# google/vizier

Measured on AMD Instinct MI355X. Metric: suggest_wall_clock_ms_gp_bandit_20d_n1000, lower is better.
Workload: dtype fp32; 1 GPU; model=gp_bandit_matern52_ucb_eagle, dim=20, n_trials=1000, acquisition_evals_per_gpu=75000, eagle_batch=25, ard=warm_lbfgs_12it_x2, global_batch=1, parallelism=dp1_sharded_sweep

## Files before the change

### vizier_amd/_src/ops/csrc/eagle_sweep.hip

```cpp

#include <hip/hip_runtime.h>

#include "common.h"

#define BLOCK 256
#define MAX_POOL 128
#define SWEEP_NCHUNK 10
#define POOL_LDS_CAP 8192
#define RESIDENT_CAP (POOL_LDS_CAP / 2)

__device__ __forceinline__ float cload(const float* p) {
  return __hip_atomic_load(p, __ATOMIC_RELAXED, __HIP_MEMORY_SCOPE_AGENT);
}
__device__ __forceinline__ void cstore(float* p, float v) {
  __hip_atomic_store(p, v, __ATOMIC_RELAXED, __HIP_MEMORY_SCOPE_AGENT);
}

__device__ __forceinline__ void grid_sync(unsigned int* bar,
                                          unsigned int& target) {
  __builtin_amdgcn_s_waitcnt(0);
  __syncthreads();
  target += gridDim.x;
  if (threadIdx.x == 0) {
    asm volatile("" ::: "memory");
    const unsigned int count = __hip_atomic_fetch_add(
        bar, 1u, __ATOMIC_RELAXED, __HIP_MEMORY_SCOPE_AGENT) + 1u;
    if ((int)(count - target) < 0) {
      while ((int)(__hip_atomic_load(bar, __ATOMIC_RELAXED,
                                     __HIP_MEMORY_SCOPE_AGENT) -
                   target) < 0) {
        __builtin_amdgcn_s_sleep(8);
      }
    }
    asm volatile("" ::: "memory");
  }
  __syncthreads();
}

#define FOLD_MAX_TILES 1024

__device__ __forceinline__ void reduce_all_partials(
    const float* var_ws, int batch_size, int total_tiles, float* wp) {
  const int tid = threadIdx.x;
  float sacc[VZ_QF_QMAX];
#pragma unroll
  for (int q = 0; q < VZ_QF_QMAX; ++q) sacc[q] = 0.0f;
  for (int w0 = 0; w0 < total_tiles; w0 += BLOCK) {
    const int w = w0 + tid;
    const bool live = w < total_tiles;
    const int wc = live ? w : total_tiles - 1;
    float v[VZ_QF_QMAX];
#pragma unroll
    for (int q = 0; q < VZ_QF_QMAX; ++q) {
      const int qc = min(q, batch_size - 1);
      v[q] = cload(var_ws + (long)qc * (total_tiles + 1) + wc);
    }
#pragma unroll
    for (int q = 0; q < VZ_QF_QMAX; ++q) {
      sacc[q] = live ? sacc[q] + v[q] : sacc[q];
    }
  }
  const int lane = tid & (WAVE_SIZE - 1);
#pragma unroll
  for (int off = WAVE_SIZE / 2; off > 1; off >>= 1) {
    const bool up = (lane & off) != 0;
#pragma unroll
    for (int i = 0; i < off / 2; ++i) {
      const float keep = up ? sacc[2 * i + 1] : sacc[2 * i];
      const float send = up ? sacc[2 * i] : sacc[2 * i + 1];
      sacc[i] = keep + __shfl_xor(send, off, WAVE_SIZE);
    }
  }
  const float total = sacc[0] + __shfl_xor(sacc[0], 1, WAVE_SIZE);
  if ((lane & 1) == 0) {
    const int q = (int)(__brev((unsigned)(lane >> 1)) >> 27);
    wp[(tid / WAVE_SIZE) * VZ_QF_QMAX + q] = total;
  }
}

__device__ __forceinline__ float fold_quad(const float* wp, int q) {
  return (wp[q] + wp[2 * VZ_QF_QMAX + q]) +
         (wp[VZ_QF_QMAX + q] + wp[3 * VZ_QF_QMAX + q]);
}

template <typename LoadK, typename StoreP>
__device__ __forceinline__ void vz_quadform_tile_pipelined(
    const float* __restrict__ kinv, int b, int n, int tile, int tiles_n,
    float* k_i_lds, float* k_j_lds, LoadK loadk, StoreP store,
    unsigned long long* prof = nullptr) {
  constexpr int kStage = VZ_QF_QMAX * VZ_QF_TILE / BLOCK;
  const int tid = threadIdx.x;
  const bool profme = (prof != nullptr && tid == 0);
  unsigned long long tq0 = profme ? wall_clock64() : 0;
  const int ti = tile / tiles_n, tj = tile % tiles_n;
  const int i0 = ti * VZ_QF_TILE, j0 = tj * VZ_QF_TILE;
  const int ilen = min(VZ_QF_TILE, n - i0);
  const int jlen = min(VZ_QF_TILE, n - j0);
  {
    const int c = tid % VZ_QF_TILE;
    const int q0 = tid / VZ_QF_TILE;
    const int ci = i0 + min(c, ilen - 1), cj = j0 + min(c, jlen - 1);
    float ri[kStage], rj[kStage];
#pragma unroll
    for (int u = 0; u < kStage; ++u) {
      const long base =
          (long)min(q0 + u * (BLOCK / VZ_QF_TILE), b - 1) * n;
      ri[u] = loadk(base + ci);
      rj[u] = loadk(base + cj);
    }
#pragma unroll
    for (int u = 0; u < kStage; ++u) {
      const bool inq = q0 + u * (BLOCK / VZ_QF_TILE) < b;
      k_i_lds[tid + u * BLOCK] = (inq && c < ilen) ? ri[u] : 0.0f;
      k_j_lds[tid + u * BLOCK] = (inq && c < jlen) ? rj[u] : 0.0f;
    }
  }
  __syncthreads();
  if (profme) {
    const unsigned long long tq1 = wall_clock64();
    prof[0] += tq1 - tq0;
    tq0 = tq1;
  }
  const int wave = tid / WAVE_SIZE;
  const int lane = tid % WAVE_SIZE;
  float acc[8];
#pragma unroll
  for (int qq = 0; qq < 8; ++qq) acc[qq] = 0.0f;
  if (lane < jlen) {
    if (ilen == VZ_QF_TILE) {
      for (int ib = 0; ib < VZ_QF_TILE; ib += 8) {
        float kvv[8];
#pragma unroll
        for (int u = 0; u < 8; ++u) {
          kvv[u] = kinv[(long)(i0 + ib + u) * n + j0 + lane];
        }
#pragma unroll
        for (int u = 0; u < 8; ++u) {
#pragma unroll
          for (int qq = 0; qq < 8; ++qq) {
            acc[qq] = fmaf(
                k_i_lds[(wave * 8 + qq) * VZ_QF_TILE + ib + u],
                kvv[u], acc[qq]);
          }
        }
      }
    } else {
      for (int i = 0; i < ilen; ++i) {
        const float kv = kinv[(long)(i0 + i) * n + j0 + lane];
#pragma unroll
        for (int qq = 0; qq < 8; ++qq) {
          acc[qq] = fmaf(k_i_lds[(wave * 8 + qq) * VZ_QF_TILE + i], kv,
                         acc[qq]);
        }
      }
    }
  }
#pragma unroll
  for (int qq = 0; qq < 8; ++qq) {
    const int q = wave * 8 + qq;
    float v = acc[qq] * k_j_lds[q * VZ_QF_TILE + lane];
    v = wave_reduce_sum(v);
    if (lane == 0 && q < b) store(q, v);
  }
  __syncthreads();
  if (profme) prof[1] += wall_clock64() - tq0;
}

__device__ __forceinline__ float sweep_matern52(float d2) {
#pragma clang fp contract(off)
  const float r = sqrtf(fmaxf(d2, 0.0f));
  const float sr = 2.2360679774997896f * r;
  const float one_sr = 1.0f + sr;
  return fmaf(sr * sr, 1.0f / 3.0f, one_sr) * __expf(-sr);
}

#define KV_ROWS 4
#define KV_CHUNK 4

template <bool VEC4>
__device__ __forceinline__ void sweep_kvec(
    const float* __restrict__ x, const float* __restrict__ inv_ls,
    const float* __restrict__ alpha, const float* xq_lds, float* k_row,
    int dc, int n, float amp2, float& mu_acc, float& min_linf) {
  for (int row0 = threadIdx.x; row0 < n; row0 += KV_ROWS * BLOCK) {
    const float* xr[KV_ROWS];
    float al[KV_ROWS];
#pragma unroll
    for (int s = 0; s < KV_ROWS; ++s) {
      const int rc = min(row0 + s * BLOCK, n - 1);
      xr[s] = x + (long)rc * dc;
      al[s] = alpha[rc];
    }
    auto load_chunk = [&](float (&buf)[KV_ROWS][KV_CHUNK], int j0) {
#pragma unroll
      for (int s = 0; s < KV_ROWS; ++s) {
        if (VEC4) {
          const float4 v = *reinterpret_cast<const float4*>(xr[s] + j0);
          buf[s][0] = v.x; buf[s][1] = v.y; buf[s][2] = v.z; buf[s][3] = v.w;
        } else {
#pragma unroll
          for (int c = 0; c < KV_CHUNK; ++c) {
            buf[s][c] = xr[s][min(j0 + c, dc - 1)];
          }
        }
      }
    };
    float d2[KV_ROWS], linf[KV_ROWS];
#pragma unroll
    for (int s = 0; s < KV_ROWS; ++s) d2[s] = linf[s] = 0.0f;
    for (int j0 = 0; j0 < dc; j0 += KV_CHUNK) {
      float cur[KV_ROWS][KV_CHUNK];
      load_chunk(cur, j0);
      float xq[KV_CHUNK], il[KV_CHUNK];
#pragma unroll
      for (int c = 0; c < KV_CHUNK; ++c) {
        const int jc = VEC4 ? j0 + c : min(j0 + c, dc - 1);
        xq[c] = xq_lds[jc];
        il[c] = inv_ls[jc];
      }
#pragma unroll
      for (int c = 0; c < KV_CHUNK; ++c) {
        if (VEC4 || j0 + c < dc) {
#pragma unroll
          for (int s = 0; s < KV_ROWS; ++s) {
            const float diff = xq[c] - cur[s][c];
            const float z = diff * il[c];
            d2[s] = fmaf(z, z, d2[s]);
            linf[s] = fmaxf(linf[s], fabsf(diff));
          }
        }
      }
    }
#pragma unroll
    for (int s = 0; s < KV_ROWS; ++s) {
      const int row = row0 + s * BLOCK;
      const bool live = row < n;
      const float kv = amp2 * sweep_matern52(d2[s]);
      if (live) cstore(k_row + row, kv);
      mu_acc = live ? fmaf(kv, al[s], mu_acc) : mu_acc;
      min_linf = live ? fminf(min_linf, linf[s]) : min_linf;
    }
  }
}

extern "C" __global__ __launch_bounds__(BLOCK) void
eagle_sweep_kernel(
    float* __restrict__ pool_cont,
    float* __restrict__ rewards,
    float* __restrict__ perturbations,
    float* __restrict__ best_reward,
    unsigned long long* __restrict__ iter_ptr,
    unsigned int* __restrict__ barrier_buf,
    const float* __restrict__ x,
    const float* __restrict__ inv_ls,
    const float* __restrict__ alpha,
    const float* __restrict__ kinv,
    float* __restrict__ out_cont,
    float* __restrict__ k_ws,
    float* __restrict__ mu_ws,
    float* __restrict__ dist_ws,
    float* __restrict__ var_ws,
    float* __restrict__ slot_ws,
    int n_batches, int batch_size, int pool_size, int dc, int n,
    long long it_start, long long iterations,
    float visibility, float gravity, float neg_gravity, float norm_scale,
    float penalize_factor, float perturbation_lower_bound,
    float base_perturbation,
    unsigned long long seed_suggest, unsigned long long seed_update,
    float amp2, float mean_c, int acq, float coef, float best_value,
    float tr_radius) {
  __shared__ float scale[MAX_POOL];
  __shared__ float red[8];
  __shared__ float s_scalar;
  __shared__ __attribute__((aligned(16))) float xq_lds[512];
  __shared__ float pool_lds[POOL_LDS_CAP];
  __shared__ float st_rewards[MAX_POOL];
  __shared__ float st_perts[MAX_POOL];
  __shared__ float st_best;

  const int tid = threadIdx.x;
  const int G = gridDim.x;
  const int pool_elems = pool_size * dc;
  const bool resident = pool_elems <= RESIDENT_CAP;
  const bool stage_pool = !resident && pool_elems <= POOL_LDS_CAP;
  const bool pool_in_lds = resident || stage_pool;
  const bool owner = blockIdx.x < batch_size;
  const bool x_vec4 = dc % KV_CHUNK == 0 &&
                      (reinterpret_cast<unsigned long long>(x) & 15) == 0;
  float* st_pool = pool_lds + RESIDENT_CAP;
  const float* pl = resident ? st_pool : pool_lds;
  auto fsum = [](float a, float c) { return a + c; };
  auto fmin_ = [](float a, float c) { return fminf(a, c); };
  auto fmax_ = [](float a, float c) { return fmaxf(a, c); };

  const bool profwg = (blockIdx.x == 0 && threadIdx.x == 0);
  unsigned long long tmark = profwg ? wall_clock64() : 0;
  unsigned int bar_target = 0;
#define VZ_SWEEP_PROF(slot)                                        \
  if (profwg) {                                                    \
    const unsigned long long tnow = wall_clock64();                \
    iter_ptr[2 + (slot)] += tnow - tmark;                          \
    tmark = tnow;                                                  \
  }

  if (resident && owner) {
    for (int e = tid; e < pool_elems; e += BLOCK) st_pool[e] = pool_cont[e];
    for (int p = tid; p < pool_size; p += BLOCK) {
      st_rewards[p] = rewards[p];
      st_perts[p] = perturbations[p];
    }
    if (tid == 0) st_best = best_reward[0];
    __syncthreads();
  }

  for (long long it = it_start; it < it_start + iterations; ++it) {
    const unsigned long long offset = (unsigned long long)it;
    float* slot_c = slot_ws + (long)(it & 1) * batch_size * (dc + 2);
    float* slot_mu = slot_c + batch_size * dc;
    float* slot_dist = slot_mu + batch_size;
    const int batch_start =
        (int)(offset % (unsigned long long)n_batches) * batch_size;
    if (profwg) tmark = wall_clock64();

    for (int b = blockIdx.x; b < batch_size; b += G) {
      if (stage_pool) {
        for (int e = tid; e < pool_elems; e += BLOCK) {
          pool_lds[e] = cload(pool_cont + e);
        }
        __syncthreads();
      }
      const int me = batch_start + b;
      const float my_reward = resident ? st_rewards[me]
                                       : cload(rewards + me);
      const float my_pert = resident ? st_perts[me]
                                     : cload(perturbations + me);
      for (int p = tid; p < pool_size; p += BLOCK) {
        float d2 = 0.0f;
        if (pool_in_lds) {
          for (int j = 0; j < dc; ++j) {
            const float diff = pl[me * dc + j] - pl[p * dc + j];
            d2 = fmaf(diff, diff, d2);
          }
        } else {
          for (int j = 0; j < dc; ++j) {
            const float diff = cload(pool_cont + me * dc + j) -
                               cload(pool_cont + p * dc + j);
            d2 = fmaf(diff, diff, d2);
          }
        }
        const float reward_p = resident ? st_rewards[p]
                                        : cload(rewards + p);
        const float dir = (reward_p - my_reward >= 0.0f) ? gravity
                                                         : -neg_gravity;
        const float force = __expf(-visibility * d2 / dc * 10.0f);
        float s = dir * force;
        if (!isfinite(reward_p)) s = 0.0f;
        scale[p] = s;
      }
      __syncthreads();
      float pulls = 0.0f, pushes = 0.0f;
      for (int p = tid; p < pool_size; p += BLOCK) {
        pulls += (scale[p] > 0.0f) ? 1.0f : 0.0f;
        pushes += (scale[p] < 0.0f) ? 1.0f : 0.0f;
      }
      float n_pull = block_reduce(pulls, red, fsum, 0.0f);
      if (tid == 0) red[4] = fmaxf(n_pull, 1.0f);
      __syncthreads();
      float n_push = block_reduce(pushes, red, fsum, 0.0f);
      if (tid == 0) red[5] = fmaxf(n_push, 1.0f);
      __syncthreads();
      const float inv_pull = 1.0f / red[4];
      const float inv_push = 1.0f / red[5];
      float ssum = 0.0f;
      for (int p = tid; p < pool_size; p += BLOCK) {
        const float s = scale[p];
        const float ns = norm_scale * (s > 0.0f ? s * inv_pull
                                                : s * inv_push);
        scale[p] = ns;
        ssum += ns;
      }
      __syncthreads();
      float scale_sum = block_reduce(ssum, red, fsum, 0.0f);
      if (tid == 0) s_scalar = scale_sum;
      __syncthreads();
      scale_sum = s_scalar;
      for (int j = tid; j < dc; j += BLOCK) {
        float moved = 0.0f;
        if (pool_in_lds) {
          for (int p = 0; p < pool_size; ++p) {
            moved = fmaf(scale[p], pl[p * dc + j], moved);
          }
        } else {
          for (int p = 0; p < pool_size; ++p) {
            moved = fmaf(scale[p], cload(pool_cont + p * dc + j), moved);
          }
        }
        const float mine = pool_in_lds ? pl[me * dc + j]
                                       : cload(pool_cont + me * dc + j);
        moved = mine + (moved - mine * scale_sum);
        float noise = vz_rng_laplace<float>(seed_suggest, offset,
                                     (unsigned)(b * dc + j));
        noise = (noise >= 0.0f) ? 1.0f : -1.0f;
        const float cand = moved + noise * my_pert;
        out_cont[b * dc + j] = cand;
        if (resident) cstore(slot_c + b * dc + j, cand);
        xq_lds[j] = cand;
      }
      __syncthreads();

      float mu_acc = 0.0f;
      float min_linf = INFINITY;
      if (x_vec4) {
        sweep_kvec<true>(x, inv_ls, alpha, xq_lds, k_ws + (long)b * n, dc,
                         n, amp2, mu_acc, min_linf);
      } else {
        sweep_kvec<false>(x, inv_ls, alpha, xq_lds, k_ws + (long)b * n, dc,
                          n, amp2, mu_acc, min_linf);
      }
      float mu = block_reduce(mu_acc, red, fsum, 0.0f);
      if (tid == 0) {
        cstore(mu_ws + b, mu);
        if (resident) cstore(slot_mu + b, mu);
      }
      __syncthreads();
      float dist = block_reduce(min_linf, red, fmin_, INFINITY);
      if (tid == 0) {
        cstore(dist_ws + b, dist);
        if (resident) cstore(slot_dist + b, dist);
      }
      __syncthreads();
    }
    VZ_SWEEP_PROF(0)
    grid_sync(barrier_buf, bar_target);
    VZ_SWEEP_PROF(1)

    {
      const int tiles_n = (n + VZ_QF_TILE - 1) / VZ_QF_TILE;
      const int total_tiles = tiles_n * tiles_n;
      float* k_i_lds = pool_lds;
      float* k_j_lds = pool_lds + VZ_QF_QMAX * VZ_QF_TILE;
      for (int tile = blockIdx.x; tile < total_tiles; tile += G) {
        const int t = tile;
        vz_quadform_tile_pipelined(
            kinv, batch_size, n, t, tiles_n, k_i_lds, k_j_lds,
            [&](long idx) { return cload(k_ws + idx); },
            [&](int q, float v) {
              cstore(var_ws + (long)q * (total_tiles + 1) + t, v);
            },
            blockIdx.x == 0 ? iter_ptr + 10 : nullptr);
      }
    }
    VZ_SWEEP_PROF(2)
    grid_sync(barrier_buf, bar_target);
    VZ_SWEEP_PROF(3)

    const int tiles_n_c = (n + VZ_QF_TILE - 1) / VZ_QF_TILE;
    const int total_tiles_c = tiles_n_c * tiles_n_c;
    const bool fold = total_tiles_c <= FOLD_MAX_TILES;
    if (!fold) {
      for (int q = blockIdx.x; q < batch_size; q += G) {
        float sacc = 0.0f;
        for (int w = tid; w < total_tiles_c; w += BLOCK) {
          sacc += cload(var_ws + (long)q * (total_tiles_c + 1) + w);
        }
        float total = block_reduce(sacc, red, fsum, 0.0f);
        if (tid == 0) {
          cstore(var_ws + (long)q * (total_tiles_c + 1) + total_tiles_c,
                 total);
        }
        __syncthreads();
      }
      VZ_SWEEP_PROF(4)
      grid_sync(barrier_buf, bar_target);
      VZ_SWEEP_PROF(5)
    }

    float* wp = pool_lds;
    float* sc_lds = pool_lds + 4 * VZ_QF_QMAX;
    auto score_of = [&](float quad, float mu_raw, float dist) {
      float var = fmaxf(amp2 - quad, 1e-12f);
      const float sd = sqrtf(var);
      const float mu = mu_raw + mean_c;
      return vz_trust_region(vz_acq_score(acq, mu, sd, coef, best_value),
                             dist, tr_radius);
    };
    if (resident) {
      if (owner) {
        float mu_t = 0.0f, dist_t = 0.0f;
        if (tid < batch_size) {
          mu_t = cload(slot_mu + tid);
          dist_t = cload(slot_dist + tid);
        }
        if (fold) {
          reduce_all_partials(var_ws, batch_size, total_tiles_c, wp);
        }
        __syncthreads();
        if (tid < WAVE_SIZE) {
          float score = -INFINITY;
          if (tid < batch_size) {
            float* reduced =
                var_ws + (long)tid * (total_tiles_c + 1) + total_tiles_c;
            float quad;
            if (fold) {
              quad = fold_quad(wp, tid);
              if (tid % G == (int)blockIdx.x) cstore(reduced, quad);
            } else {
              quad = cload(reduced);
            }
            score = score_of(quad, mu_t, dist_t);
            sc_lds[tid] = score;
          }
          const float batch_max = wave_reduce_max(score);
          if (tid == 0) s_scalar = fmaxf(st_best, batch_max);
        }
        __syncthreads();
        const float new_best = s_scalar;
        for (int e = tid; e < batch_size * dc; e += BLOCK) {
          const int i = e / dc;
          const int me = batch_start + i;
          const int ej = me * dc + (e - i * dc);
          const float new_r = sc_lds[i];
          const float old_r = st_rewards[me];
          const bool improved = new_r > old_r;
          const float old_pert = st_perts[me];
          const float pert = improved ? old_pert
                                      : old_pert * penalize_factor;
          const float reward = improved ? new_r : old_r;
          const bool dead = (pert < perturbation_lower_bound) &&
                            (reward != new_best);
          if (dead) {
            st_pool[ej] = vz_rng_uniform<float>(
                seed_update, offset ^ 0x5151ull, (unsigned)ej);
          } else if (improved) {
            st_pool[ej] = cload(slot_c + e);
          }
        }
        __syncthreads();
        if (tid < batch_size) {
          const int me = batch_start + tid;
          const float new_r = sc_lds[tid];
          const float old_r = st_rewards[me];
          const bool improved = new_r > old_r;
          const float old_pert = st_perts[me];
          float pert = improved ? old_pert : old_pert * penalize_factor;
          float reward = improved ? new_r : old_r;
          const bool dead = (pert < perturbation_lower_bound) &&
                            (reward != new_best);
          if (dead) {
            reward = -INFINITY;
            pert = base_perturbation;
          }
          st_rewards[me] = reward;
          st_perts[me] = pert;
        }
        if (tid == 0) st_best = new_best;
        __syncthreads();
      }
      VZ_SWEEP_PROF(6)
    } else {
      if (fold && owner) {
        reduce_all_partials(var_ws, batch_size, total_tiles_c, wp);
        __syncthreads();
      }
      for (int i = blockIdx.x; i < batch_size; i += G) {
        float local_max = -INFINITY;
        float my_score = -INFINITY;
        for (int t = tid; t < batch_size; t += BLOCK) {
          float* reduced =
              var_ws + (long)t * (total_tiles_c + 1) + total_tiles_c;
          float quad;
          if (fold) {
            quad = fold_quad(wp, t);
            if (t == i) cstore(reduced, quad);
          } else {
            quad = cload(reduced);
          }
          const float score =
              score_of(quad, cload(mu_ws + t), cload(dist_ws + t));
          local_max = fmaxf(local_max, score);
          if (t == i) my_score = score;
        }
        float batch_max = block_reduce(local_max, red, fmax_, -INFINITY);
        if (tid == (i % BLOCK) && i < BLOCK) red[6] = my_score;
        __syncthreads();
        const float new_r = red[6];
        if (tid == 0) {
          s_scalar = fmaxf(cload(best_reward), batch_max);
          if (i == 0) cstore(best_reward, s_scalar);
        }
        __syncthreads();
        const float new_best = s_scalar;
        const int me = batch_start + i;
        const float old_r = cload(rewards + me);
        const bool improved = new_r > old_r;
        const float old_pert = cload(perturbations + me);
        float pert = improved ? old_pert : old_pert * penalize_factor;
        float reward = improved ? new_r : old_r;
        const bool dead = (pert < perturbation_lower_bound) &&
                          (reward != new_best);
        if (improved) {
          for (int j = tid; j < dc; j += BLOCK) {
            cstore(pool_cont + me * dc + j, out_cont[i * dc + j]);
          }
        }
        if (dead) {
          for (int j = tid; j < dc; j += BLOCK) {
            cstore(pool_cont + me * dc + j,
                   vz_rng_uniform<float>(seed_update, offset ^ 0x5151ull,
                                  (unsigned)(me * dc + j)));
          }
          reward = -INFINITY;
          pert = base_perturbation;
        }
        if (tid == 0) {
          cstore(rewards + me, reward);
          cstore(perturbations + me, pert);
        }
        __syncthreads();
      }
      VZ_SWEEP_PROF(6)
      grid_sync(barrier_buf, bar_target);
      VZ_SWEEP_PROF(7)
    }
  }

  if (resident && blockIdx.x == 0 && iterations > 0) {
    for (int e = tid; e < pool_elems; e += BLOCK) {
      cstore(pool_cont + e, st_pool[e]);
    }
    for (int p = tid; p < pool_size; p += BLOCK) {
      cstore(rewards + p, st_rewards[p]);
      cstore(perturbations + p, st_perts[p]);
    }
    if (tid == 0) cstore(best_reward, st_best);
  }

  if (blockIdx.x == 0 && tid == 0) {
    iter_ptr[0] = (unsigned long long)(it_start + iterations);
    iter_ptr[1] = (unsigned long long)(it_start + iterations - 1);
  }
}

extern "C" int launch_eagle_sweep(
    float* pool_cont, float* rewards, float* perturbations,
    float* best_reward, unsigned long long* iter_ptr,
    unsigned int* barrier_buf, const float* x, const float* inv_ls,
    const float* alpha, const float* kinv, float* out_cont, float* k_ws,
    float* mu_ws, float* dist_ws, float* var_ws, float* slot_ws,
    int n_batches,
    int batch_size, int pool_size, int dc, int n, long long it_start,
    long long iterations, float visibility, float gravity,
    float neg_gravity, float norm_scale, float penalize_factor,
    float perturbation_lower_bound, float base_perturbation,
    unsigned long long seed_suggest, unsigned long long seed_update,
    float amp2, float mean_c, int acq, float coef, float best_value,
    float tr_radius, hipStream_t stream) {
  int dev = 0;
  (void)hipGetDevice(&dev);
  int coop = 0;
  (void)hipDeviceGetAttribute(&coop, hipDeviceAttributeCooperativeLaunch,
                              dev);
  if (!coop) return 0;
  int num_cu = 0;
  (void)hipDeviceGetAttribute(&num_cu,
                              hipDeviceAttributeMultiprocessorCount, dev);
  int blocks_per_cu = 0;
  hipError_t err = hipOccupancyMaxActiveBlocksPerMultiprocessor(
      &blocks_per_cu, (const void*)eagle_sweep_kernel, BLOCK, 0);
  if (err != hipSuccess || blocks_per_cu < 1) return 0;
  const int tiles_n = (n + VZ_QF_TILE - 1) / VZ_QF_TILE;
  int grid = tiles_n * tiles_n;
  if (grid > 128) grid = 128;
  if (grid < 64) grid = 64;
  static int grid_env = -1;
  if (grid_env < 0) {
    const char* env = getenv("VIZIER_AMD_SWEEP_GRID");
    grid_env = (env != nullptr) ? atoi(env) : 0;
  }
  if (grid_env > 0) grid = grid_env;
  const int max_grid = blocks_per_cu * num_cu;
  if (grid > max_grid) grid = max_grid;
  if (grid < 1) grid = 1;

  void* args[] = {
      &pool_cont, &rewards, &perturbations, &best_reward, &iter_ptr,
      &barrier_buf, &x, &inv_ls, &alpha, &kinv, &out_cont, &k_ws,
      &mu_ws, &dist_ws, &var_ws, &slot_ws, &n_batches, &batch_size, &pool_size,
      &dc, &n, &it_start, &iterations, &visibility, &gravity,
      &neg_gravity, &norm_scale, &penalize_factor,
      &perturbation_lower_bound, &base_perturbation, &seed_suggest,
      &seed_update, &amp2, &mean_c, &acq, &coef, &best_value,
      &tr_radius};
  err = hipLaunchCooperativeKernel((const void*)eagle_sweep_kernel,
                                   dim3(grid), dim3(BLOCK), args, 0,
                                   stream);
  if (err != hipSuccess) return -(int)err;
  return grid;
}
```

Before: 148.6 ms.

## Double sweep block size so two halves process quadform tiles concurrently

Launches the cooperative sweep kernel with 512 threads per block. The second half of each block sits idle in most phases, but in the quadform stage it processes a separate tile using its own LDS staging buffer, which doubles tile throughput per block. Paired block reductions are also merged into one pass, and the pool distance and move loops are chunked so loads can be issued together. The cost is higher register and LDS pressure and many idle threads in the other phases. The merged reductions rely on only the first 256 threads contributing, so correctness depends on that guard holding.

```diff
diff --git a/vizier_amd/_src/ops/csrc/eagle_sweep.hip b/vizier_amd/_src/ops/csrc/eagle_sweep.hip
--- a/vizier_amd/_src/ops/csrc/eagle_sweep.hip
+++ b/vizier_amd/_src/ops/csrc/eagle_sweep.hip
@@ -4,6 +4,8 @@
 #include "common.h"
 
 #define BLOCK 256
+#define SWEEP_THREADS (2 * BLOCK)
+#define SWEEP_IDLE (1 << 30)
 #define MAX_POOL 128
 #define SWEEP_NCHUNK 10
 #define POOL_LDS_CAP 8192
@@ -37,6 +39,53 @@
   __syncthreads();
 }
 
+template <typename T, typename Op>
+__device__ __forceinline__ T sweep_block_reduce(T v, T* lds4, Op op,
+                                                T init) {
+  const int lane = threadIdx.x & (WAVE_SIZE - 1);
+  const int wave = threadIdx.x / WAVE_SIZE;
+#pragma unroll
+  for (int offset = WAVE_SIZE / 2; offset > 0; offset >>= 1) {
+    v = op(v, __shfl_down(v, offset, WAVE_SIZE));
+  }
+  if (lane == 0 && wave < BLOCK / WAVE_SIZE) lds4[wave] = v;
+  __syncthreads();
+  if (wave == 0) {
+    v = (lane < BLOCK / WAVE_SIZE) ? lds4[lane] : init;
+#pragma unroll
+    for (int offset = 2; offset > 0; offset >>= 1) {
+      v = op(v, __shfl_down(v, offset, WAVE_SIZE));
+    }
+  }
+  return v;
+}
+
+template <typename T, typename Op1, typename Op2>
+__device__ __forceinline__ void sweep_block_reduce2(
+    T& v1, T& v2, T* lds4a, T* lds4b, Op1 op1, Op2 op2, T init1, T init2) {
+  const int lane = threadIdx.x & (WAVE_SIZE - 1);
+  const int wave = threadIdx.x / WAVE_SIZE;
+#pragma unroll
+  for (int offset = WAVE_SIZE / 2; offset > 0; offset >>= 1) {
+    v1 = op1(v1, __shfl_down(v1, offset, WAVE_SIZE));
+    v2 = op2(v2, __shfl_down(v2, offset, WAVE_SIZE));
+  }
+  if (lane == 0 && wave < BLOCK / WAVE_SIZE) {
+    lds4a[wave] = v1;
+    lds4b[wave] = v2;
+  }
+  __syncthreads();
+  if (wave == 0) {
+    v1 = (lane < BLOCK / WAVE_SIZE) ? lds4a[lane] : init1;
+    v2 = (lane < BLOCK / WAVE_SIZE) ? lds4b[lane] : init2;
+#pragma unroll
+    for (int offset = 2; offset > 0; offset >>= 1) {
+      v1 = op1(v1, __shfl_down(v1, offset, WAVE_SIZE));
+      v2 = op2(v2, __shfl_down(v2, offset, WAVE_SIZE));
+    }
+  }
+}
+
 #define FOLD_MAX_TILES 1024
 
 __device__ __forceinline__ void reduce_all_partials(
@@ -86,17 +135,16 @@
 template <typename LoadK, typename StoreP>
 __device__ __forceinline__ void vz_quadform_tile_pipelined(
     const float* __restrict__ kinv, int b, int n, int tile, int tiles_n,
-    float* k_i_lds, float* k_j_lds, LoadK loadk, StoreP store,
-    unsigned long long* prof = nullptr) {
+    int tid, bool live, float* k_i_lds, float* k_j_lds, LoadK loadk,
+    StoreP store, unsigned long long* prof = nullptr) {
   constexpr int kStage = VZ_QF_QMAX * VZ_QF_TILE / BLOCK;
-  const int tid = threadIdx.x;
-  const bool profme = (prof != nullptr && tid == 0);
+  const bool profme = (prof != nullptr && threadIdx.x == 0);
   unsigned long long tq0 = profme ? wall_clock64() : 0;
   const int ti = tile / tiles_n, tj = tile % tiles_n;
   const int i0 = ti * VZ_QF_TILE, j0 = tj * VZ_QF_TILE;
   const int ilen = min(VZ_QF_TILE, n - i0);
   const int jlen = min(VZ_QF_TILE, n - j0);
-  {
+  if (live) {
     const int c = tid % VZ_QF_TILE;
     const int q0 = tid / VZ_QF_TILE;
     const int ci = i0 + min(c, ilen - 1), cj = j0 + min(c, jlen - 1);
@@ -121,46 +169,48 @@
     prof[0] += tq1 - tq0;
     tq0 = tq1;
   }
-  const int wave = tid / WAVE_SIZE;
-  const int lane = tid % WAVE_SIZE;
-  float acc[8];
-#pragma unroll
-  for (int qq = 0; qq < 8; ++qq) acc[qq] = 0.0f;
-  if (lane < jlen) {
-    if (ilen == VZ_QF_TILE) {
-      for (int ib = 0; ib < VZ_QF_TILE; ib += 8) {
-        float kvv[8];
-#pragma unroll
-        for (int u = 0; u < 8; ++u) {
-          kvv[u] = kinv[(long)(i0 + ib + u) * n + j0 + lane];
-        }
-#pragma unroll
-        for (int u = 0; u < 8; ++u) {
+  if (live) {
+    const int wave = tid / WAVE_SIZE;
+    const int lane = tid % WAVE_SIZE;
+    float acc[8];
+#pragma unroll
+    for (int qq = 0; qq < 8; ++qq) acc[qq] = 0.0f;
+    if (lane < jlen) {
+      if (ilen == VZ_QF_TILE) {
+        for (int ib = 0; ib < VZ_QF_TILE; ib += 8) {
+          float kvv[8];
+#pragma unroll
+          for (int u = 0; u < 8; ++u) {
+            kvv[u] = kinv[(long)(i0 + ib + u) * n + j0 + lane];
+          }
+#pragma unroll
+          for (int u = 0; u < 8; ++u) {
+#pragma unroll
+            for (int qq = 0; qq < 8; ++qq) {
+              acc[qq] = fmaf(
+                  k_i_lds[(wave * 8 + qq) * VZ_QF_TILE + ib + u],
+                  kvv[u], acc[qq]);
+            }
+          }
+        }
+      } else {
+        for (int i = 0; i < ilen; ++i) {
+          const float kv = kinv[(long)(i0 + i) * n + j0 + lane];
 #pragma unroll
           for (int qq = 0; qq < 8; ++qq) {
-            acc[qq] = fmaf(
-                k_i_lds[(wave * 8 + qq) * VZ_QF_TILE + ib + u],
-                kvv[u], acc[qq]);
-          }
-        }
-      }
-    } else {
-      for (int i = 0; i < ilen; ++i) {
-        const float kv = kinv[(long)(i0 + i) * n + j0 + lane];
-#pragma unroll
-        for (int qq = 0; qq < 8; ++qq) {
-          acc[qq] = fmaf(k_i_lds[(wave * 8 + qq) * VZ_QF_TILE + i], kv,
-                         acc[qq]);
-        }
-      }
-    }
-  }
-#pragma unroll
-  for (int qq = 0; qq < 8; ++qq) {
-    const int q = wave * 8 + qq;
-    float v = acc[qq] * k_j_lds[q * VZ_QF_TILE + lane];
-    v = wave_reduce_sum(v);
-    if (lane == 0 && q < b) store(q, v);
+            acc[qq] = fmaf(k_i_lds[(wave * 8 + qq) * VZ_QF_TILE + i], kv,
+                           acc[qq]);
+          }
+        }
+      }
+    }
+#pragma unroll
+    for (int qq = 0; qq < 8; ++qq) {
+      const int q = wave * 8 + qq;
+      float v = acc[qq] * k_j_lds[q * VZ_QF_TILE + lane];
+      v = wave_reduce_sum(v);
+      if (lane == 0 && q < b) store(q, v);
+    }
   }
   __syncthreads();
   if (profme) prof[1] += wall_clock64() - tq0;
@@ -176,13 +226,15 @@
 
 #define KV_ROWS 4
 #define KV_CHUNK 4
+#define SG_DCHUNK 8
+#define SG_PCHUNK 16
 
 template <bool VEC4>
 __device__ __forceinline__ void sweep_kvec(
     const float* __restrict__ x, const float* __restrict__ inv_ls,
     const float* __restrict__ alpha, const float* xq_lds, float* k_row,
-    int dc, int n, float amp2, float& mu_acc, float& min_linf) {
-  for (int row0 = threadIdx.x; row0 < n; row0 += KV_ROWS * BLOCK) {
+    int dc, int n, int wt, float amp2, float& mu_acc, float& min_linf) {
+  for (int row0 = wt; row0 < n; row0 += KV_ROWS * BLOCK) {
     const float* xr[KV_ROWS];
     float al[KV_ROWS];
 #pragma unroll
@@ -243,7 +295,7 @@
   }
 }
 
-extern "C" __global__ __launch_bounds__(BLOCK) void
+extern "C" __global__ __launch_bounds__(SWEEP_THREADS) void
 eagle_sweep_kernel(
     float* __restrict__ pool_cont,
     float* __restrict__ rewards,
@@ -271,14 +323,19 @@
     float tr_radius) {
   __shared__ float scale[MAX_POOL];
   __shared__ float red[8];
+  __shared__ float red2[4];
   __shared__ float s_scalar;
   __shared__ __attribute__((aligned(16))) float xq_lds[512];
   __shared__ float pool_lds[POOL_LDS_CAP];
+  __shared__ float stage1_lds[2 * VZ_QF_QMAX * VZ_QF_TILE];
   __shared__ float st_rewards[MAX_POOL];
   __shared__ float st_perts[MAX_POOL];
   __shared__ float st_best;
 
   const int tid = threadIdx.x;
+  const int half = tid / BLOCK;
+  const int htid = tid % BLOCK;
+  const int wt = half == 0 ? tid : SWEEP_IDLE;
   const int G = gridDim.x;
   const int pool_elems = pool_size * dc;
   const bool resident = pool_elems <= RESIDENT_CAP;
@@ -304,8 +361,8 @@
   }
 
   if (resident && owner) {
-    for (int e = tid; e < pool_elems; e += BLOCK) st_pool[e] = pool_cont[e];
-    for (int p = tid; p < pool_size; p += BLOCK) {
+    for (int e = wt; e < pool_elems; e += BLOCK) st_pool[e] = pool_cont[e];
+    for (int p = wt; p < pool_size; p += BLOCK) {
       st_rewards[p] = rewards[p];
       st_perts[p] = perturbations[p];
     }
@@ -324,7 +381,7 @@
 
     for (int b = blockIdx.x; b < batch_size; b += G) {
       if (stage_pool) {
-        for (int e = tid; e < pool_elems; e += BLOCK) {
+        for (int e = wt; e < pool_elems; e += BLOCK) {
           pool_lds[e] = cload(pool_cont + e);
         }
         __syncthreads();
@@ -334,20 +391,28 @@
                                        : cload(rewards + me);
       const float my_pert = resident ? st_perts[me]
                                      : cload(perturbations + me);
-      for (int p = tid; p < pool_size; p += BLOCK) {
+      auto dist2 = [&](auto ld, int p) {
         float d2 = 0.0f;
-        if (pool_in_lds) {
-          for (int j = 0; j < dc; ++j) {
-            const float diff = pl[me * dc + j] - pl[p * dc + j];
-            d2 = fmaf(diff, diff, d2);
-          }
-        } else {
-          for (int j = 0; j < dc; ++j) {
-            const float diff = cload(pool_cont + me * dc + j) -
-                               cload(pool_cont + p * dc + j);
-            d2 = fmaf(diff, diff, d2);
-          }
-        }
+        for (int j0 = 0; j0 < dc; j0 += SG_DCHUNK) {
+          float mv[SG_DCHUNK], pv[SG_DCHUNK];
+#pragma unroll
+          for (int u = 0; u < SG_DCHUNK; ++u) {
+            const int jc = min(j0 + u, dc - 1);
+            mv[u] = ld(me * dc + jc);
+            pv[u] = ld(p * dc + jc);
+          }
+#pragma unroll
+          for (int u = 0; u < SG_DCHUNK; ++u) {
+            const float diff = mv[u] - pv[u];
+            d2 = (j0 + u < dc) ? fmaf(diff, diff, d2) : d2;
+          }
+        }
+        return d2;
+      };
+      auto ld_lds = [&](int idx) { return pl[idx]; };
+      auto ld_mem = [&](int idx) { return cload(pool_cont + idx); };
+      for (int p = wt; p < pool_size; p += BLOCK) {
+        const float d2 = pool_in_lds ? dist2(ld_lds, p) : dist2(ld_mem, p);
         const float reward_p = resident ? st_rewards[p]
                                         : cload(rewards + p);
         const float dir = (reward_p - my_reward >= 0.0f) ? gravity
@@ -359,20 +424,20 @@
       }
       __syncthreads();
       float pulls = 0.0f, pushes = 0.0f;
-      for (int p = tid; p < pool_size; p += BLOCK) {
+      for (int p = wt; p < pool_size; p += BLOCK) {
         pulls += (scale[p] > 0.0f) ? 1.0f : 0.0f;
         pushes += (scale[p] < 0.0f) ? 1.0f : 0.0f;
       }
-      float n_pull = block_reduce(pulls, red, fsum, 0.0f);
-      if (tid == 0) red[4] = fmaxf(n_pull, 1.0f);
-      __syncthreads();
-      float n_push = block_reduce(pushes, red, fsum, 0.0f);
-      if (tid == 0) red[5] = fmaxf(n_push, 1.0f);
+      sweep_block_reduce2(pulls, pushes, red, red2, fsum, fsum, 0.0f, 0.0f);
+      if (tid == 0) {
+        red[4] = fmaxf(pulls, 1.0f);
+        red[5] = fmaxf(pushes, 1.0f);
+      }
       __syncthreads();
       const float inv_pull = 1.0f / red[4];
       const float inv_push = 1.0f / red[5];
       float ssum = 0.0f;
-      for (int p = tid; p < pool_size; p += BLOCK) {
+      for (int p = wt; p < pool_size; p += BLOCK) {
         const float s = scale[p];
         const float ns = norm_scale * (s > 0.0f ? s * inv_pull
                                                 : s * inv_push);
@@ -380,21 +445,31 @@
         ssum += ns;
       }
       __syncthreads();
-      float scale_sum = block_reduce(ssum, red, fsum, 0.0f);
+      float scale_sum = sweep_block_reduce(ssum, red, fsum, 0.0f);
       if (tid == 0) s_scalar = scale_sum;
       __syncthreads();
       scale_sum = s_scalar;
-      for (int j = tid; j < dc; j += BLOCK) {
+      auto moved_of = [&](auto ld, int j) {
         float moved = 0.0f;
-        if (pool_in_lds) {
-          for (int p = 0; p < pool_size; ++p) {
-            moved = fmaf(scale[p], pl[p * dc + j], moved);
-          }
-        } else {
-          for (int p = 0; p < pool_size; ++p) {
-            moved = fmaf(scale[p], cload(pool_cont + p * dc + j), moved);
-          }
-        }
+        for (int p0 = 0; p0 < pool_size; p0 += SG_PCHUNK) {
+          float sv[SG_PCHUNK], pv[SG_PCHUNK];
+#pragma unroll
+          for (int u = 0; u < SG_PCHUNK; ++u) {
+            const int pc = min(p0 + u, pool_size - 1);
+            sv[u] = scale[pc];
+            pv[u] = ld(pc * dc + j);
+          }
+#pragma unroll
+          for (int u = 0; u < SG_PCHUNK; ++u) {
+            moved = (p0 + u < pool_size) ? fmaf(sv[u], pv[u], moved)
+                                         : moved;
+          }
+        }
+        return moved;
+      };
+      for (int j = wt; j < dc; j += BLOCK) {
+        float moved = pool_in_lds ? moved_of(ld_lds, j)
+                                  : moved_of(ld_mem, j);
         const float mine = pool_in_lds ? pl[me * dc + j]
                                        : cload(pool_cont + me * dc + j);
         moved = mine + (moved - mine * scale_sum);
@@ -412,21 +487,20 @@
       float min_linf = INFINITY;
       if (x_vec4) {
         sweep_kvec<true>(x, inv_ls, alpha, xq_lds, k_ws + (long)b * n, dc,
-                         n, amp2, mu_acc, min_linf);
+                         n, wt, amp2, mu_acc, min_linf);
       } else {
         sweep_kvec<false>(x, inv_ls, alpha, xq_lds, k_ws + (long)b * n, dc,
-                          n, amp2, mu_acc, min_linf);
-      }
-      float mu = block_reduce(mu_acc, red, fsum, 0.0f);
+                          n, wt, amp2, mu_acc, min_linf);
+      }
+      sweep_block_reduce2(mu_acc, min_linf, red, red2, fsum, fmin_, 0.0f,
+                          INFINITY);
       if (tid == 0) {
-        cstore(mu_ws + b, mu);
-        if (resident) cstore(slot_mu + b, mu);
-      }
-      __syncthreads();
-      float dist = block_reduce(min_linf, red, fmin_, INFINITY);
-      if (tid == 0) {
-        cstore(dist_ws + b, dist);
-        if (resident) cstore(slot_dist + b, dist);
+        cstore(mu_ws + b, mu_acc);
+        cstore(dist_ws + b, min_linf);
+        if (resident) {
+          cstore(slot_mu + b, mu_acc);
+          cstore(slot_dist + b, min_linf);
+        }
       }
       __syncthreads();
     }
@@ -437,12 +511,13 @@
     {
       const int tiles_n = (n + VZ_QF_TILE - 1) / VZ_QF_TILE;
       const int total_tiles = tiles_n * tiles_n;
-      float* k_i_lds = pool_lds;
-      float* k_j_lds = pool_lds + VZ_QF_QMAX * VZ_QF_TILE;
-      for (int tile = blockIdx.x; tile < total_tiles; tile += G) {
-        const int t = tile;
+      float* k_i_lds = half == 0 ? pool_lds : stage1_lds;
+      float* k_j_lds = k_i_lds + VZ_QF_QMAX * VZ_QF_TILE;
+      for (int tile0 = blockIdx.x; tile0 < total_tiles; tile0 += 2 * G) {
+        const int t = tile0 + half * G;
         vz_quadform_tile_pipelined(
-            kinv, batch_size, n, t, tiles_n, k_i_lds, k_j_lds,
+            kinv, batch_size, n, t, tiles_n, htid, t < total_tiles,
+            k_i_lds, k_j_lds,
             [&](long idx) { return cload(k_ws + idx); },
             [&](int q, float v) {
               cstore(var_ws + (long)q * (total_tiles + 1) + t, v);
@@ -460,10 +535,10 @@
     if (!fold) {
       for (int q = blockIdx.x; q < batch_size; q += G) {
         float sacc = 0.0f;
-        for (int w = tid; w < total_tiles_c; w += BLOCK) {
+        for (int w = wt; w < total_tiles_c; w += BLOCK) {
           sacc += cload(var_ws + (long)q * (total_tiles_c + 1) + w);
         }
-        float total = block_reduce(sacc, red, fsum, 0.0f);
+        float total = sweep_block_reduce(sacc, red, fsum, 0.0f);
         if (tid == 0) {
           cstore(var_ws + (long)q * (total_tiles_c + 1) + total_tiles_c,
                  total);
@@ -491,7 +566,7 @@
           mu_t = cload(slot_mu + tid);
           dist_t = cload(slot_dist + tid);
         }
-        if (fold) {
+        if (fold && half == 0) {
           reduce_all_partials(var_ws, batch_size, total_tiles_c, wp);
         }
         __syncthreads();
@@ -515,7 +590,7 @@
         }
         __syncthreads();
         const float new_best = s_scalar;
-        for (int e = tid; e < batch_size * dc; e += BLOCK) {
+        for (int e = wt; e < batch_size * dc; e += BLOCK) {
           const int i = e / dc;
           const int me = batch_start + i;
           const int ej = me * dc + (e - i * dc);
@@ -559,13 +634,15 @@
       VZ_SWEEP_PROF(6)
     } else {
       if (fold && owner) {
-        reduce_all_partials(var_ws, batch_size, total_tiles_c, wp);
+        if (half == 0) {
+          reduce_all_partials(var_ws, batch_size, total_tiles_c, wp);
+        }
         __syncthreads();
       }
       for (int i = blockIdx.x; i < batch_size; i += G) {
         float local_max = -INFINITY;
         float my_score = -INFINITY;
-        for (int t = tid; t < batch_size; t += BLOCK) {
+        for (int t = wt; t < batch_size; t += BLOCK) {
           float* reduced =
               var_ws + (long)t * (total_tiles_c + 1) + total_tiles_c;
           float quad;
@@ -580,7 +657,7 @@
           local_max = fmaxf(local_max, score);
           if (t == i) my_score = score;
         }
-        float batch_max = block_reduce(local_max, red, fmax_, -INFINITY);
+        float batch_max = sweep_block_reduce(local_max, red, fmax_, -INFINITY);
         if (tid == (i % BLOCK) && i < BLOCK) red[6] = my_score;
         __syncthreads();
         const float new_r = red[6];
@@ -599,12 +676,12 @@
         const bool dead = (pert < perturbation_lower_bound) &&
                           (reward != new_best);
         if (improved) {
-          for (int j = tid; j < dc; j += BLOCK) {
+          for (int j = wt; j < dc; j += BLOCK) {
             cstore(pool_cont + me * dc + j, out_cont[i * dc + j]);
           }
         }
         if (dead) {
-          for (int j = tid; j < dc; j += BLOCK) {
+          for (int j = wt; j < dc; j += BLOCK) {
             cstore(pool_cont + me * dc + j,
                    vz_rng_uniform<float>(seed_update, offset ^ 0x5151ull,
                                   (unsigned)(me * dc + j)));
@@ -625,10 +702,10 @@
   }
 
   if (resident && blockIdx.x == 0 && iterations > 0) {
-    for (int e = tid; e < pool_elems; e += BLOCK) {
+    for (int e = wt; e < pool_elems; e += BLOCK) {
       cstore(pool_cont + e, st_pool[e]);
     }
-    for (int p = tid; p < pool_size; p += BLOCK) {
+    for (int p = wt; p < pool_size; p += BLOCK) {
       cstore(rewards + p, st_rewards[p]);
       cstore(perturbations + p, st_perts[p]);
     }
@@ -666,7 +743,7 @@
                               hipDeviceAttributeMultiprocessorCount, dev);
   int blocks_per_cu = 0;
   hipError_t err = hipOccupancyMaxActiveBlocksPerMultiprocessor(
-      &blocks_per_cu, (const void*)eagle_sweep_kernel, BLOCK, 0);
+      &blocks_per_cu, (const void*)eagle_sweep_kernel, SWEEP_THREADS, 0);
   if (err != hipSuccess || blocks_per_cu < 1) return 0;
   const int tiles_n = (n + VZ_QF_TILE - 1) / VZ_QF_TILE;
   int grid = tiles_n * tiles_n;
@@ -692,7 +769,7 @@
       &seed_update, &amp2, &mean_c, &acq, &coef, &best_value,
       &tr_radius};
   err = hipLaunchCooperativeKernel((const void*)eagle_sweep_kernel,
-                                   dim3(grid), dim3(BLOCK), args, 0,
+                                   dim3(grid), dim3(SWEEP_THREADS), args, 0,
                                    stream);
   if (err != hipSuccess) return -(int)err;
   return grid;
```

Result: faster. 132.9 ms, median of 6 (-10.5%).
